# GemsLab/H2GCN

Hardware: AMD Instinct MI355X
Metric: aggregated edges/sec (1+2-hop SpMM) (higher is better)
Workload: dtype f32

## Files before the change

h2gcn_amd/csrc/spmm_kernels.hip.h:

```cpp
#pragma once

#include <hip/hip_runtime.h>
#include <stdint.h>

#include <type_traits>

#include "h2gcn_hip.h"

namespace h2gcn {

constexpr int kWave = 64;
constexpr int kWavesPerBlock = 4;
constexpr int kBlock = kWave * kWavesPerBlock;
constexpr int kNumXcd = 8;
constexpr int kMaxRowsPerWave = 7;
#ifndef H2GCN_MIN_WAVES
#define H2GCN_MIN_WAVES 6
#endif
constexpr int kMinWavesPerSimd = H2GCN_MIN_WAVES;
#ifndef H2GCN_SHORT_MIN_WAVES
#define H2GCN_SHORT_MIN_WAVES 4
#endif
#ifndef H2GCN_SHORT_FB4_MIN_WAVES
#define H2GCN_SHORT_FB4_MIN_WAVES 7
// ... 158 lines not shown
}

template <int VEC, int LPR, int NP>
__device__ __forceinline__ void fold_tree(const float (&acc)[NP][VEC], float (&tot)[VEC]) {
    constexpr int G = kWave / LPR;
    static_assert(NP == Tree<LPR>::NP, "partials per lane");
#pragma unroll
    for (int i = 0; i < VEC; ++i) {
        if constexpr (G == 1) tot[i] = (acc[0][i] + acc[1][i]) + (acc[2][i] + acc[3][i]);
        else if constexpr (G == 2) tot[i] = fold_xor32(acc[0][i]) + fold_xor32(acc[1][i]);
        else tot[i] = fold_groups<LPR>(acc[0][i]);
    }
}

template <int VEC, int NP>
__device__ __forceinline__ void zero_acc(float (&acc)[NP][VEC]) {
#pragma unroll
    for (int k = 0; k < NP; ++k)
#pragma unroll
        for (int i = 0; i < VEC; ++i) acc[k][i] = 0.f;
}

template <typename TS, int VEC>
__device__ __forceinline__ typename LoadT<TS, VEC>::type load_vec(const void* p) {
#ifdef H2GCN_NT_GATHER
    return __builtin_nontemporal_load(reinterpret_cast<const typename LoadT<TS, VEC>::type*>(p));
#else
    return *reinterpret_cast<const typename LoadT<TS, VEC>::type*>(p);
#endif
}

template <typename TS, int VEC>
__device__ __forceinline__ typename LoadT<TS, VEC>::type zero_load() {
    if constexpr (std::is_same<TS, float>::value && VEC > 1) return (typename VecT<VEC>::type)(0.f);
    else return (typename LoadT<TS, VEC>::type)0;
}

template <typename TS, int VEC>
__device__ __forceinline__ void fma_vec(float (&acc)[VEC], float w, typename LoadT<TS, VEC>::type x) {
    if constexpr (std::is_same<TS, bf16>::value) {
        if constexpr (VEC == 1) {
            acc[0] = fmaf(w, __uint_as_float((uint32_t)x << 16), acc[0]);
        } else if constexpr (VEC == 2) {
            acc[0] = fmaf(w, bf16_lo(x), acc[0]);
            acc[1] = fmaf(w, bf16_hi(x), acc[1]);
        } else {
#pragma unroll
            for (int i = 0; i < VEC / 2; ++i) {
                acc[2 * i] = fmaf(w, bf16_lo(x[i]), acc[2 * i]);
                acc[2 * i + 1] = fmaf(w, bf16_hi(x[i]), acc[2 * i + 1]);
            }
        }
    } else if constexpr (VEC == 1) {
        acc[0] = fmaf(w, x, acc[0]);
    } else {
#pragma unroll
        for (int i = 0; i < VEC; ++i) acc[i] = fmaf(w, x[i], acc[i]);
    }
}

template <bool OFF32>
struct GatherAddr {
    const char* base;
    typename std::conditional<OFF32, uint32_t, int64_t>::type lane_off;
    typename std::conditional<OFF32, uint32_t, int64_t>::type ld_bytes;
    __device__ __forceinline__ const void* row(int col) const {
        if constexpr (OFF32) {
            return base + (uint32_t)(lane_off + (uint32_t)col * ld_bytes);
        } else {
            return base + (lane_off + (int64_t)col * ld_bytes);
        }
    }
};

template <typename TS, int VEC, int LPR, int U, bool PREDICATED, bool OFF32, int PHASE = 0, int NP>
__device__ __forceinline__ void gather_batch(int c, float v, int t, int g, const GatherAddr<OFF32>& addr, bool take,
                                             float (&acc)[NP][VEC]) {
    constexpr int G = kWave / LPR;
    typename LoadT<TS, VEC>::type x[U];
    float w[U];
#pragma unroll
    for (int u = 0; u < U; ++u) {
        int cj;
        if constexpr (G == 1) {
            cj = __builtin_amdgcn_readlane(c, t + u);
            w[u] = __int_as_float(__builtin_amdgcn_readlane(__float_as_int(v), t + u));
        } else {
            const int idx = ((t + u) * G + g) & (kWave - 1);
            cj = lane_gather(c, idx);
            w[u] = lane_gather(v, idx);
        }
        const void* p = addr.row(cj);
        if constexpr (PREDICATED) {
            if (take) {
                x[u] = load_vec<TS, VEC>(p);
            } else {
                w[u] = 0.f;
                x[u] = zero_load<TS, VEC>();
            }
        } else {
            x[u] = load_vec<TS, VEC>(p);
        }
    }
#pragma unroll
    for (int u = 0; u < U; ++u) fma_vec<TS, VEC>(acc[(PHASE + u) % NP], w[u], x[u]);
}

__device__ __forceinline__ void load_chunk(const int32_t* __restrict__ colidx, const float* __restrict__ vals,
                                           int64_t base, int64_t seg_end, int lane, int& c, float& v) {
    c = 0;
    v = 0.f;
    if (base + lane < seg_end) {
        c = __builtin_nontemporal_load(colidx + base + lane);
        v = __builtin_nontemporal_load(vals + base + lane);
    }
}

template <typename TS, int VEC, int LPR, bool MASKED, bool OFF32, int MAXB = H2GCN_MAIN_MAXB, int NP>
__device__ __forceinline__ void process_chunk(int c, float v, int n, int g, const GatherAddr<OFF32>& addr,
                                              bool lane_active, float (&acc)[NP][VEC]) {
    constexpr int G = kWave / LPR;
    const int full = n / G;
    int t = 0;
    if constexpr (MAXB >= 8)
        for (; t + 8 <= full; t += 8) gather_batch<TS, VEC, LPR, 8, MASKED, OFF32>(c, v, t, g, addr, lane_active, acc);
    if constexpr (MAXB < 8)
        for (; t + 4 <= full; t += 4) gather_batch<TS, VEC, LPR, 4, MASKED, OFF32>(c, v, t, g, addr, lane_active, acc);
    if (t + 4 <= full) {
        gather_batch<TS, VEC, LPR, 4, MASKED, OFF32>(c, v, t, g, addr, lane_active, acc);
        t += 4;
    }
    const int rem = n - full * G;
    if (t + 2 <= full) {
        gather_batch<TS, VEC, LPR, 2, MASKED, OFF32>(c, v, t, g, addr, lane_active, acc);
        t += 2;
        if (t + 1 <= full) {
            gather_batch<TS, VEC, LPR, 1, MASKED, OFF32, 2 % NP>(c, v, t, g, addr, lane_active, acc);
            if constexpr (G > 1)
                if (rem > 0) gather_batch<TS, VEC, LPR, 1, true, OFF32, 3 % NP>(c, v, full, g, addr, lane_active && g < rem, acc);
        } else {
            if constexpr (G > 1)
                if (rem > 0) gather_batch<TS, VEC, LPR, 1, true, OFF32, 2 % NP>(c, v, full, g, addr, lane_active && g < rem, acc);
        }
    } else if (t + 1 <= full) {
        gather_batch<TS, VEC, LPR, 1, MASKED, OFF32>(c, v, t, g, addr, lane_active, acc);
        if constexpr (G > 1)
            if (rem > 0) gather_batch<TS, VEC, LPR, 1, true, OFF32, 1 % NP>(c, v, full, g, addr, lane_active && g < rem, acc);
    } else {
        if constexpr (G > 1)
            if (rem > 0) gather_batch<TS, VEC, LPR, 1, true, OFF32>(c, v, full, g, addr, lane_active && g < rem, acc);
    }
}

template <typename TS, int VEC, int LPR, bool MASKED, bool OFF32, int MAXB = H2GCN_MAIN_MAXB, int NP>
__device__ __forceinline__ void accumulate_segment(const int32_t* __restrict__ colidx,
                                                   const float* __restrict__ vals, int64_t seg_begin,
                                                   int64_t seg_end, int chunk0, int chunk_step,
                                                   const GatherAddr<OFF32>& addr, int lane, bool lane_active,
                                                   float (&acc)[NP][VEC]) {
    const int g = lane / LPR;
    for (int64_t base = seg_begin + (int64_t)chunk0 * kWave; base < seg_end; base += (int64_t)chunk_step * kWave) {
        const int64_t left = seg_end - base;
        const int n = left < kWave ? (int)left : kWave;
        int c;
        float v;
        load_chunk(colidx, vals, base, seg_end, lane, c, v);
        process_chunk<TS, VEC, LPR, MASKED, OFF32, MAXB>(c, v, n, g, addr, lane_active, acc);
    }
}

template <typename TS, int VEC, int LPR, bool OFF32, int MAXB = H2GCN_MAIN_MAXB, int NP>
__device__ __forceinline__ void accumulate_segment_prefetched(const int32_t* __restrict__ colidx,
                                                              const float* __restrict__ vals, int64_t seg_begin,
                                                              int64_t seg_end, int c, float v,
                                                              const GatherAddr<OFF32>& addr, int lane,
                                                              float (&acc)[NP][VEC]) {
    const int g = lane / LPR;
    for (int64_t base = seg_begin; base < seg_end; base += kWave) {
        const int64_t left = seg_end - base;
        const int n = left < kWave ? (int)left : kWave;
        int c_next = 0;
        float v_next = 0.f;
        if (left > kWave) load_chunk(colidx, vals, base + kWave, seg_end, lane, c_next, v_next);
        process_chunk<TS, VEC, LPR, false, OFF32, MAXB>(c, v, n, g, addr, true, acc);
        c = c_next;
        v = v_next;
    }
}

template <typename TS, int VEC, int LPR, bool OFF32>
__device__ __forceinline__ void accumulate_grouped(int c, float v, int n_mine, int n_max, int lane,
                                                   const GatherAddr<OFF32>& addr, float (&part)[kTreeParts][VEC]) {
    constexpr int U = kTreeParts;
    const int group_base = lane & ~(LPR - 1);
    for (int t = 0; t < n_max; t += U) {
        typename LoadT<TS, VEC>::type x[U];
        float w[U];
#pragma unroll
        for (int u = 0; u < U; ++u) {
            const int cj = lane_gather(c, group_base + t + u);
            w[u] = lane_gather(v, group_base + t + u);
            if (t + u < n_mine) {
                x[u] = load_vec<TS, VEC>(addr.row(cj));
            } else {
                w[u] = 0.f;
                x[u] = zero_load<TS, VEC>();
            }
        }
#pragma unroll
        for (int u = 0; u < U; ++u)
            if (t + u < n_mine) fma_vec<TS, VEC>(part[u], w[u], x[u]);
    }
}

template <int VEC>
__device__ __forceinline__ void combine_partials(const float (&part)[kTreeParts][VEC], float (&acc)[VEC]) {
#pragma unroll
    for (int i = 0; i < VEC; ++i) acc[i] = (part[0][i] + part[1][i]) + (part[2][i] + part[3][i]);
}

__device__ __forceinline__ float relu_keep_nan(float t) { return t < 0.f ? 0.f : t; }

template <int VEC>
__device__ __forceinline__ void epilogue(float (&acc)[VEC], const float* __restrict__ bias, int relu, int col) {
    if (bias) {
#pragma unroll
        for (int i = 0; i < VEC; ++i) acc[i] += bias[col + i];
    }
    if (relu) {
#pragma unroll
        for (int i = 0; i < VEC; ++i) acc[i] = relu_keep_nan(acc[i]);
    }
}

template <typename TD>
__device__ __forceinline__ void store_one(TD* p, float t) {
    if constexpr (std::is_same<TD, bf16>::value)
        __builtin_nontemporal_store(__builtin_bit_cast(uint16_t, (__bf16)t), reinterpret_cast<uint16_t*>(p));
    else
        __builtin_nontemporal_store(t, p);
}

template <typename TD, int VEC>
__device__ __forceinline__ void store_vec(TD* p, const float (&acc)[VEC]) {
    if constexpr (std::is_same<TD, bf16>::value) {
        if constexpr (VEC == 1) {
            store_one<TD>(p, acc[0]);
        } else if constexpr (VEC == 2) {
            __builtin_nontemporal_store(pack_bf16x2(acc[0], acc[1]), reinterpret_cast<uint32_t*>(p));
        } else {
            typename LoadT<bf16, VEC>::type o;
#pragma unroll
            for (int i = 0; i < VEC / 2; ++i) o[i] = pack_bf16x2(acc[2 * i], acc[2 * i + 1]);
            __builtin_nontemporal_store(o, reinterpret_cast<typename LoadT<bf16, VEC>::type*>(p));
        }
    } else if constexpr (VEC == 1) {
        __builtin_nontemporal_store(acc[0], p);
    } else {
        typename VecT<VEC>::type o;
#pragma unroll
        for (int i = 0; i < VEC; ++i) o[i] = acc[i];
#if defined(H2GCN_AB_NO_STORES)
        if (acc[0] == 1.2345678e30f)
            __builtin_nontemporal_store(o, reinterpret_cast<typename VecT<VEC>::type*>(p));
#elif defined(H2GCN_PLAIN_STORES)
        *reinterpret_cast<typename VecT<VEC>::type*>(p) = o;
#else
        __builtin_nontemporal_store(o, reinterpret_cast<typename VecT<VEC>::type*>(p));
#endif
    }
}

template <typename TD, int VEC, bool GEN, typename P>
__device__ __forceinline__ void store_out(const P& p, TD* row, int col0, int ecol, float (&tot)[VEC]) {
    constexpr bool kF32 = std::is_same<TD, float>::value;
    if (col0 + VEC <= p.d) {
        if constexpr (GEN) {
            if (kF32 && p.accumulate) {
                if constexpr (VEC == 1) {
                    tot[0] += reinterpret_cast<const float*>(row)[col0];
                } else {
                    const typename VecT<VEC>::type old = *reinterpret_cast<const typename VecT<VEC>::type*>(reinterpret_cast<const float*>(row) + col0);
#pragma unroll
                    for (int i = 0; i < VEC; ++i) tot[i] += old[i];
                }
            }
            epilogue<VEC>(tot, p.bias, p.relu, col0);
        }
        store_vec<TD, VEC>(row + col0, tot);
        return;
    }
    if constexpr (GEN) {
        if (col0 < p.d) {
#pragma unroll
            for (int i = 0; i < VEC; ++i) {
                const int c = ecol + i;
                if (c >= col0 && c < p.d) {
                    float t = tot[i];
                    if (kF32 && p.accumulate) t += reinterpret_cast<const float*>(row)[c];
                    if (p.bias) t += p.bias[c];
                    if (p.relu) t = relu_keep_nan(t);
                    store_one<TD>(row + c, t);
                }
            }
        }
    }
// ... 165 lines not shown
__device__ __forceinline__ void in_tile_short_rows(const LaunchParams& p, int lane, int rpw, int64_t row0, int rows_here, int rp_lo, int rp_hi,
                                                   int64_t lane_off0_, int64_t src_col_begin, int lcol, int ecol) {
    using off_t = typename std::conditional<OFF32, uint32_t, int64_t>::type;
    constexpr int NP = Tree<LPR>::NP;
    constexpr int kBias = VEC;
    const int li = lane % LPR, g = lane / LPR;
    const int n_sel = p.n_sel;
    const off_t lane_off0 = (off_t)lane_off0_;
    auto seg_bound = [&](int l) -> int64_t {
        return ((int64_t)__builtin_amdgcn_readlane(rp_hi, l) << 32) | (uint32_t)__builtin_amdgcn_readlane(rp_lo, l);
    };
    {
        constexpr int G = kWave / LPR;
        const int short_max = min(LPR, p.long_threshold - 1);
        const int n_blocks = (rows_here + G - 1) / G;
        const GatherAddr<OFF32> addr0{nullptr, lane_off0, (off_t)(p.ld_src * sizeof(TS))};
        auto row_wave_wide = [&](int r, int s_first, int s_last) {
            float acc[NP][VEC];
            zero_acc<VEC, NP>(acc);
            if constexpr (SUM) {
                for (int s = s_first; s < s_last; ++s) {
                    const int l0 = s * (rpw + 1) + r;
                    if (seg_bound(l0 + 1) - seg_bound(l0) >= p.long_threshold) return;
                }
            }
            for (int s = s_first; s < s_last; ++s) {
                const int l0 = s * (rpw + 1) + r;
                const int64_t sb = seg_bound(l0), se = seg_bound(l0 + 1);
                if (!SUM && se - sb >= p.long_threshold) continue;
                const HopCsr& h = p.hop[s];
                GatherAddr<OFF32> addr = addr0;
                addr.base = reinterpret_cast<const char*>(src_ptr<TS>(p.src) + p.src_hop_off[s] + src_col_begin - kBias);
                accumulate_segment<TS, VEC, LPR, false, OFF32, FB>(h.colidx, h.vals, sb, se, 0, 1, addr, lane, true, acc);
                if constexpr (!SUM) {
                    float tot[VEC];
                    fold_tree<VEC, LPR, NP>(acc, tot);
                    if (g == 0) store_out<TD, VEC, EPI>(p, dst_ptr<TD>(p.dst) + (row0 + r) * p.ld_dst + p.dst_hop_off[s], lcol, ecol, tot);
                    zero_acc<VEC, NP>(acc);
                }
            }
            if constexpr (SUM) {
                float tot[VEC];
                fold_tree<VEC, LPR, NP>(acc, tot);
                if (g == 0) store_out<TD, VEC, EPI>(p, dst_ptr<TD>(p.dst) + (row0 + r) * p.ld_dst, lcol, ecol, tot);
            }
        };
        auto my_segment = [&](int s, int blk, int64_t& begin, int& len) {
            const int r = blk * G + g;
            const int l0 = s * (rpw + 1) + min(r, rpw - 1);
            const int64_t sb = ((int64_t)lane_gather(rp_hi, l0) << 32) | (uint32_t)lane_gather(rp_lo, l0);
            const int64_t se = ((int64_t)lane_gather(rp_hi, l0 + 1) << 32) | (uint32_t)lane_gather(rp_lo, l0 + 1);
            begin = sb;
            const int64_t n = se - sb;
            len = r < rows_here ? (int)(n > 0x7fffffff ? 0x7fffffff : n) : -1;
        };
        if constexpr (!SUM) {
            const int n_rounds = n_sel * n_blocks;
            int64_t begin_n = 0;
            int len_n = -1, c_n = 0;
            float v_n = 0.f;
            bool short_n = false;
            auto fetch = [&](int i) {
                const int s_ = i / n_blocks, blk_ = i - s_ * n_blocks;
                my_segment(s_, blk_, begin_n, len_n);
                short_n = __builtin_amdgcn_ballot_w64(len_n > short_max) == 0;
                c_n = 0;
                v_n = 0.f;
                if (short_n && li < len_n) {
                    c_n = __builtin_nontemporal_load(p.hop[s_].colidx + begin_n + li);
                    v_n = __builtin_nontemporal_load(p.hop[s_].vals + begin_n + li);
                }
            };
            if (n_rounds > 0) fetch(0);
            for (int i = 0; i < n_rounds; ++i) {
                const int s = i / n_blocks, blk = i - s * n_blocks;
                const int len = len_n, c = c_n;
                const float v = v_n;
                const bool is_short = short_n;
                if (i + 1 < n_rounds) fetch(i + 1);
                if (is_short) {
                    int n_max = 0;
#pragma unroll
                    for (int gg = 0; gg < G; ++gg) n_max = max(n_max, __builtin_amdgcn_readlane(len, gg * LPR));
                    float part[kTreeParts][VEC];
                    zero_acc<VEC, kTreeParts>(part);
                    GatherAddr<OFF32> addr = addr0;
                    addr.base = reinterpret_cast<const char*>(src_ptr<TS>(p.src) + p.src_hop_off[s] + src_col_begin - kBias);
                    accumulate_grouped<TS, VEC, LPR, OFF32>(c, v, len, n_max, lane, addr, part);
                    float tot[VEC];
                    combine_partials<VEC>(part, tot);
                    if (len >= 0) store_out<TD, VEC, EPI>(p, dst_ptr<TD>(p.dst) + (row0 + blk * G + g) * p.ld_dst + p.dst_hop_off[s], lcol, ecol, tot);
                } else {
                    for (int gg = 0; gg < G && blk * G + gg < rows_here; ++gg) row_wave_wide(blk * G + gg, s, s + 1);
                }
            }
        } else {
            auto block_short = [&](int blk_) {
                bool ok = true;
                for (int s_ = 0; s_ < n_sel; ++s_) {
                    int64_t b_;
                    int l_;
                    my_segment(s_, blk_, b_, l_);
                    ok = ok && __builtin_amdgcn_ballot_w64(l_ > short_max) == 0;
                }
                return ok;
            };
            int64_t begin_n = 0;
            int len_n = -1, c_n = 0;
            float v_n = 0.f;
            auto fetch = [&](int blk_, int s_, bool short_blk) {
                my_segment(s_, blk_, begin_n, len_n);
                c_n = 0;
                v_n = 0.f;
                if (short_blk && li < len_n) {
                    c_n = __builtin_nontemporal_load(p.hop[s_].colidx + begin_n + li);
                    v_n = __builtin_nontemporal_load(p.hop[s_].vals + begin_n + li);
                }
            };
            bool cur_short = n_blocks > 0 && block_short(0);
            if (n_blocks > 0) fetch(0, 0, cur_short);
            for (int blk = 0; blk < n_blocks; ++blk) {
                const bool nxt_short = blk + 1 < n_blocks && block_short(blk + 1);
                if (cur_short) {
                    float part[kTreeParts][VEC];
                    zero_acc<VEC, kTreeParts>(part);
                    bool valid = false;
                    for (int s = 0; s < n_sel; ++s) {
                        const int len = len_n, c = c_n;
                        const float v = v_n;
                        valid = len >= 0;
                        if (s + 1 < n_sel) fetch(blk, s + 1, true);
                        else if (blk + 1 < n_blocks) fetch(blk + 1, 0, nxt_short);
                        int n_max = 0;
#pragma unroll
                        for (int gg = 0; gg < G; ++gg) n_max = max(n_max, __builtin_amdgcn_readlane(len, gg * LPR));
                        GatherAddr<OFF32> addr = addr0;
                        addr.base = reinterpret_cast<const char*>(src_ptr<TS>(p.src) + p.src_hop_off[s] + src_col_begin - kBias);
                        accumulate_grouped<TS, VEC, LPR, OFF32>(c, v, len, n_max, lane, addr, part);
                    }
                    float tot[VEC];
                    combine_partials<VEC>(part, tot);
                    if (valid) store_out<TD, VEC, EPI>(p, dst_ptr<TD>(p.dst) + (row0 + blk * G + g) * p.ld_dst, lcol, ecol, tot);
                } else {
                    if (blk + 1 < n_blocks) fetch(blk + 1, 0, nxt_short);
                    for (int gg = 0; gg < G && blk * G + gg < rows_here; ++gg) row_wave_wide(blk * G + gg, 0, n_sel);
                }
                cur_short = nxt_short;
            }
        }
        return;
    }
}

template <int VEC, int LPR, bool EXACT, bool SUM, bool OFF32, bool PIPE, bool SHORT, bool EPI, int FB, bool LISTS, typename TS>
constexpr int min_waves_per_simd() {
    if (!EXACT) return 2;
    if (SHORT) return FB == 4 && !SUM ? H2GCN_SHORT_FB4_MIN_WAVES : H2GCN_SHORT_MIN_WAVES;
    const bool bf16_less = std::is_same<TS, bf16>::value && VEC == 4 &&
                           (LISTS ? FB == 4 && SUM && !OFF32
                                  : (OFF32 && EPI && LPR == 32) || (SUM && OFF32 && PIPE && LPR == 16) ||
                                        (!SUM && !OFF32 && !PIPE && !EPI && LPR == 16));
    if (LISTS && FB == 4) return H2GCN_SHORT_FB4_MIN_WAVES - bf16_less;
    const bool heavy = VEC == 4 && (LISTS ? (SUM && (!OFF32 || LPR >= 32)) || (!OFF32 && LPR >= 32)
                                          : !OFF32 ? EPI || LPR >= 32 || PIPE : PIPE && LPR == 32);
    if (heavy) return H2GCN_OFF64_HEAVY_MIN_WAVES - bf16_less;
    return (LPR >= 32 ? H2GCN_WIDE_MIN_WAVES : kMinWavesPerSimd) - bf16_less;
}

template <int VEC, int LPR, bool EXACT, bool SUM, bool OFF32, bool PIPE = false, bool SHORT = false, bool EPI = false, int FB = 8, bool LISTS = false,
          typename TS = float, typename TD = float>
__global__ __launch_bounds__(kBlock, (min_waves_per_simd<VEC, LPR, EXACT, SUM, OFF32, PIPE, SHORT, EPI, FB, LISTS, TS>())) void spmm_hops_kernel(const LaunchParams p) {
    static_assert(!LISTS || (EXACT && !SHORT && !PIPE && (LPR == 16 || LPR == 32)), "list-driven launches exist for 64- and 128-column slices");
    static_assert(EXACT || LPR == kWave, "column-tiled path uses the whole wave per row");
    __shared__ float partial[kWavesPerBlock][kMaxTileCols];
    using off_t = typename std::conditional<OFF32, uint32_t, int64_t>::type;
    constexpr int NP = Tree<LPR>::NP;
    constexpr int kMainB = LISTS ? FB : (LPR >= 32 ? H2GCN_WIDE_MAXB : H2GCN_MAIN_MAXB);

    const int lane = threadIdx.x & (kWave - 1);
    const int wave = wave_uniform(threadIdx.x >> 6);
    const int li = lane % LPR;
    const int g = lane / LPR;
    const int n_sel = p.n_sel;

    const int64_t bid = blockIdx.x;
    const int slice = EXACT ? (int)(bid / p.blocks_per_slice) : 0;
    const int64_t b = EXACT ? bid - (int64_t)slice * p.blocks_per_slice : bid;
    const int col_begin = EXACT ? slice * (VEC * LPR) : 0;
    const int col_end = EXACT ? col_begin + VEC * LPR : p.d;
    const int64_t src_col_begin = EXACT ? (int64_t)slice * p.src_slice_stride : 0;
    const int lcol = col_begin + li * VEC;
    const int ecol = EXACT ? ((lcol + VEC <= p.d_src) ? lcol : p.d_src - VEC) : lcol;
    const off_t lane_off0 = (off_t)((ecol - col_begin + VEC) * (int)sizeof(TS));
    constexpr int kBias = EXACT ? VEC : 0;

    if (b < p.n_long) {
        const int64_t entry = p.long_list[b];
        const int64_t row = SUM ? entry : (entry >> 4);
        const int s_first = SUM ? 0 : (int)(entry & 15);
        const int s_last = SUM ? n_sel : s_first + 1;
        for (int col0 = col_begin; col0 < col_end; col0 += VEC * LPR) {
            const bool lane_active = EXACT || (col0 + li * VEC < p.d);
            float acc[NP][VEC];
            zero_acc<VEC, NP>(acc);
            for (int s = s_first; s < s_last; ++s) {
                const HopCsr& h = p.hop[s];
                const int64_t sb = h.rowptr[row], se = h.rowptr[row + 1];
                const GatherAddr<OFF32> addr{reinterpret_cast<const char*>(src_ptr<TS>(p.src) + p.src_hop_off[s] + src_col_begin + (col0 - col_begin) - kBias),
                                             EXACT ? lane_off0 : (off_t)(li * VEC * (int)sizeof(TS)), (off_t)(p.ld_src * sizeof(TS))};
                accumulate_segment<TS, VEC, LPR, !EXACT, OFF32, kMainB>(h.colidx, h.vals, sb, se, wave, kWavesPerBlock, addr, lane,
                                                            lane_active, acc);
            }
            float tot[VEC];
            fold_tree<VEC, LPR, NP>(acc, tot);
            if (g == 0) {
                const int rel = EXACT ? ecol - col_begin : li * VEC;
                if (!EXACT || lcol < p.d_src) {
#pragma unroll
                    for (int i = 0; i < VEC; ++i)
                        if (rel + i >= 0) partial[wave][rel + i] = tot[i];
                }
            }
            __syncthreads();
            const int c = threadIdx.x;
            if (c < VEC * LPR && col0 + c < p.d) {
                float t = partial[0][c];
#pragma unroll
                for (int w = 1; w < kWavesPerBlock; ++w) t += partial[w][c];
                const int64_t off = row * p.ld_dst + (SUM ? 0 : p.dst_hop_off[s_first]) + col0 + c;
                if constexpr (EPI) {
                    if constexpr (std::is_same<TD, float>::value)
                        if (p.accumulate) t += dst_ptr<float>(p.dst)[off];
                    if (p.bias) t += p.bias[col0 + c];
                    if (p.relu) t = relu_keep_nan(t);
                }
                store_one<TD>(dst_ptr<TD>(p.dst) + off, t);
            }
            if (!EXACT) __syncthreads();
        }
        return;
    }

    const int64_t tb = b - p.n_long;
    int64_t tile;
    if constexpr (LISTS) {
        __shared__ uint64_t s_seg[kWavesPerBlock][kShortSumHops][kWave];
        __shared__ int32_t s_row[kWavesPerBlock][kWave];
        const int64_t q = tb >> 3;
        const int i8 = (int)(tb & 7);
        const int64_t n_groups = p.short_groups + p.med_groups;
        const int64_t s_before = (q * p.short_groups) / n_groups;
        if (((q + 1) * p.short_groups) / n_groups > s_before)
            short_list_blocks<TS, TD, VEC, LPR, SUM, OFF32, EPI, H2GCN_SHORT_PREFETCH>(p, s_before * kNumXcd + i8, lane, wave, (int64_t)lane_off0,
                                                                               src_col_begin, lcol, ecol, s_seg, s_row);
        else
            medium_list_blocks<TS, TD, VEC, LPR, SUM, OFF32, EPI, FB>(p, (q - s_before) * kNumXcd + i8, lane, wave, (int64_t)lane_off0,
                                                              src_col_begin, lcol, ecol);
        return;
    } else {
        tile = (tb % kNumXcd) * p.tiles_per_xcd + tb / kNumXcd;
    }
    if (tile >= p.n_tiles) return;
    const int rpw = p.rows_per_wave;
    const int64_t row0 = (tile * kWavesPerBlock + wave) * rpw;
    if (row0 >= p.n_rows) return;
    const int64_t rows_here_l = p.n_rows - row0;
    const int rows_here = rows_here_l < rpw ? (int)rows_here_l : rpw;

    int64_t rp = 0;
    {
        const int hs = lane / (rpw + 1), r = lane % (rpw + 1);
        if (hs < n_sel && r <= rows_here) rp = p.hop[hs].rowptr[row0 + r];
    }
    const int rp_lo = (int)(rp & 0xffffffff), rp_hi = (int)(rp >> 32);
    auto seg_bound = [&](int l) -> int64_t {
        return ((int64_t)__builtin_amdgcn_readlane(rp_hi, l) << 32) | (uint32_t)__builtin_amdgcn_readlane(rp_lo, l);
    };

    if constexpr (SHORT && EXACT && (kWave / LPR == 2 || kWave / LPR == 4)) {
        in_tile_short_rows<TS, TD, VEC, LPR, SUM, OFF32, EPI, FB>(p, lane, rpw, row0, rows_here, rp_lo, rp_hi, (int64_t)lane_off0, src_col_begin, lcol, ecol);
        return;
    }
    if constexpr (PIPE && EXACT) {
        const int n_seg = rows_here * n_sel;
        uint32_t skip = 0;
        for (int q = 0; q < n_seg; ++q) {
            const int r = q / n_sel, s_ = q - r * n_sel;
            const int l0 = s_ * (rpw + 1) + r;
            if (seg_bound(l0 + 1) - seg_bound(l0) >= p.long_threshold) skip |= SUM ? (((1u << n_sel) - 1u) << (r * n_sel)) : (1u << q);
        }
        auto seg = [&](int q, int& s_, int64_t& sb, int64_t& se) {
            const int r = q / n_sel;
            s_ = q - r * n_sel;
            const int l0 = s_ * (rpw + 1) + r;
            sb = seg_bound(l0);
            se = (skip >> q) & 1u ? sb : seg_bound(l0 + 1);
        };
        int s_cur, s_nxt = 0;
        int64_t b_cur, e_cur, b_nxt = 0, e_nxt = 0;
        int c_cur, c_nxt = 0;
        float v_cur, v_nxt = 0.f;
        seg(0, s_nxt, b_nxt, e_nxt);
        load_chunk(p.hop[s_nxt].colidx, p.hop[s_nxt].vals, b_nxt, e_nxt, lane, c_nxt, v_nxt);
        float acc[NP][VEC];
        zero_acc<VEC, NP>(acc);
        for (int q = 0; q < n_seg; ++q) {
            s_cur = s_nxt; b_cur = b_nxt; e_cur = e_nxt; c_cur = c_nxt; v_cur = v_nxt;
            if (q + 1 < n_seg) {
                seg(q + 1, s_nxt, b_nxt, e_nxt);
                load_chunk(p.hop[s_nxt].colidx, p.hop[s_nxt].vals, b_nxt, e_nxt, lane, c_nxt, v_nxt);
            }
            const int r = q / n_sel;
            const int64_t row = row0 + r;
            const HopCsr& h = p.hop[s_cur];
            const GatherAddr<OFF32> addr{reinterpret_cast<const char*>(src_ptr<TS>(p.src) + p.src_hop_off[s_cur] + src_col_begin - kBias),
                                         lane_off0, (off_t)(p.ld_src * sizeof(TS))};
            accumulate_segment_prefetched<TS, VEC, LPR, OFF32>(h.colidx, h.vals, b_cur, e_cur, c_cur, v_cur, addr, lane, acc);
            const bool skipped = (skip >> q) & 1u;
            if (!SUM || s_cur == n_sel - 1) {
                if (!skipped) {
                    float tot[VEC];
                    fold_tree<VEC, LPR, NP>(acc, tot);
                    if (g == 0) store_out<TD, VEC, EPI>(p, dst_ptr<TD>(p.dst) + row * p.ld_dst + (SUM ? 0 : p.dst_hop_off[s_cur]), lcol, ecol, tot);
                }
                zero_acc<VEC, NP>(acc);
            }
        }
        return;
    }

#ifdef H2GCN_AB_STORE_BEHIND_FETCH
    if constexpr (EXACT && !SUM && !EPI) {
        float held[VEC];
        int64_t held_off = 0;
        bool held_valid = false;
        for (int r = 0; r < rows_here; ++r) {
            const int64_t row = row0 + r;
            for (int s = 0; s < n_sel; ++s) {
                const int l0 = s * (rpw + 1) + r;
                const int64_t sb = seg_bound(l0), se = seg_bound(l0 + 1);
                if (se - sb >= p.long_threshold) continue;
                const HopCsr& h = p.hop[s];
                int c;
                float v;
                load_chunk(h.colidx, h.vals, sb, se, lane, c, v);
                if (held_valid) {
                    if (g == 0) store_out<TD, VEC, EPI>(p, dst_ptr<TD>(p.dst) + held_off, lcol, ecol, held);
                    held_valid = false;
                }
                float acc[NP][VEC];
                zero_acc<VEC, NP>(acc);
                const GatherAddr<OFF32> addr{reinterpret_cast<const char*>(src_ptr<TS>(p.src) + p.src_hop_off[s] + src_col_begin - kBias), lane_off0, (off_t)(p.ld_src * sizeof(TS))};
                accumulate_segment_prefetched<TS, VEC, LPR, OFF32, kMainB>(h.colidx, h.vals, sb, se, c, v, addr, lane, acc);
                fold_tree<VEC, LPR, NP>(acc, held);
                held_off = row * p.ld_dst + p.dst_hop_off[s];
                held_valid = true;
            }
        }
        if (held_valid && g == 0) store_out<TD, VEC, EPI>(p, dst_ptr<TD>(p.dst) + held_off, lcol, ecol, held);
        return;
    }
#endif

    for (int r = 0; r < rows_here; ++r) {
        const int64_t row = row0 + r;
        if constexpr (SUM) {
            bool skip_row = false;
            for (int s = 0; s < n_sel; ++s) {
                const int l0 = s * (rpw + 1) + r;
                const int64_t len = seg_bound(l0 + 1) - seg_bound(l0);
                if (len >= p.long_threshold) skip_row = true;
            }
            if (skip_row) continue;
        }
        for (int col0 = col_begin; col0 < col_end; col0 += VEC * LPR) {
            const bool lane_active = EXACT || (col0 + li * VEC < p.d);
            float acc[NP][VEC];
            zero_acc<VEC, NP>(acc);
#ifdef H2GCN_DEFER_HOP_STORES
            float held[VEC];
            int held_s = -1;
#endif
            for (int s = 0; s < n_sel; ++s) {
                const int l0 = s * (rpw + 1) + r;
                const int64_t sb = seg_bound(l0), se = seg_bound(l0 + 1);
                if (!SUM && se - sb >= p.long_threshold) continue;
                const HopCsr& h = p.hop[s];
                const GatherAddr<OFF32> addr{reinterpret_cast<const char*>(src_ptr<TS>(p.src) + p.src_hop_off[s] + src_col_begin + (col0 - col_begin) - kBias),
                                             EXACT ? lane_off0 : (off_t)(li * VEC * (int)sizeof(TS)), (off_t)(p.ld_src * sizeof(TS))};
                accumulate_segment<TS, VEC, LPR, !EXACT, OFF32, kMainB>(h.colidx, h.vals, sb, se, 0, 1, addr, lane, lane_active, acc);
                if constexpr (!SUM) {
                    float tot[VEC];
                    fold_tree<VEC, LPR, NP>(acc, tot);
#ifdef H2GCN_DEFER_HOP_STORES
                    if (EXACT && n_sel == 2 && s == 0) {
#pragma unroll
                        for (int i = 0; i < VEC; ++i) held[i] = tot[i];
                        held_s = 0;
                    } else {
                        if (held_s >= 0 && g == 0 && lane_active)
                            store_out<TD, VEC, EPI>(p, dst_ptr<TD>(p.dst) + row * p.ld_dst + p.dst_hop_off[held_s], lcol, ecol, held);
                        held_s = -1;
                        if (g == 0 && lane_active)
                            store_out<TD, VEC, EPI>(p, dst_ptr<TD>(p.dst) + row * p.ld_dst + p.dst_hop_off[s], EXACT ? lcol : col0 + li * VEC, EXACT ? ecol : col0 + li * VEC, tot);
                    }
#else
                    if (g == 0 && lane_active)
                        store_out<TD, VEC, EPI>(p, dst_ptr<TD>(p.dst) + row * p.ld_dst + p.dst_hop_off[s], EXACT ? lcol : col0 + li * VEC, EXACT ? ecol : col0 + li * VEC, tot);
#endif
                    zero_acc<VEC, NP>(acc);
                }
            }
#ifdef H2GCN_DEFER_HOP_STORES
            if constexpr (!SUM)
                if (held_s >= 0 && g == 0 && lane_active)
                    store_out<TD, VEC, EPI>(p, dst_ptr<TD>(p.dst) + row * p.ld_dst + p.dst_hop_off[held_s], lcol, ecol, held);
#endif
            if constexpr (SUM) {
                float tot[VEC];
                fold_tree<VEC, LPR, NP>(acc, tot);
                if (g == 0 && lane_active)
                    store_out<TD, VEC, EPI>(p, dst_ptr<TD>(p.dst) + row * p.ld_dst, EXACT ? lcol : col0 + li * VEC, EXACT ? ecol : col0 + li * VEC, tot);
            }
        }
    }
}

template <bool VEC4>
__global__ void repack_slice_major_kernel(const float* __restrict__ x, int64_t ld, int64_t ld_hop, int n_hop, int64_t n_rows,
                                          int d, int n_slices, int slice_cols, float* __restrict__ w) {
    using f4 = float __attribute__((ext_vector_type(4)));
    constexpr int E = VEC4 ? 4 : 1;
    const int cu = slice_cols / E;
    const int64_t per_hop = n_rows * cu;
// ... 95 lines not shown
```

Before: 13.73 billion.

## Stage CSR column/value indices in per-wave LDS ring for 16-lane-per-row path

Adds a per-wave shared-memory ring buffer that stages interleaved (colidx, value) pairs for up to two hops. Each block of pairs is loaded with aligned 128-bit nontemporal loads and prefetched one chunk ahead of the gather loop, replacing per-chunk global loads and readlane broadcasts of neighbour indices for LPR=16 exact, non-pipelined, non-epilogue launches. It also retunes the minimum-waves-per-SIMD heuristic for the affected variants. The ring adds LDS pressure and wave barriers, and falls back to the old path when segments are too large or more than two hops are selected.

Result: faster. 13.88 billion (median of 6 runs) (+1.1%).

```diff
diff --git a/h2gcn_amd/csrc/spmm_kernels.hip.h b/h2gcn_amd/csrc/spmm_kernels.hip.h
--- a/h2gcn_amd/csrc/spmm_kernels.hip.h
+++ b/h2gcn_amd/csrc/spmm_kernels.hip.h
@@ -334,6 +334,86 @@
     }
 }
 
+constexpr int kRingHops = 2;
+constexpr int kRingCap = 256;
+constexpr int kRingBlock = 128;
+constexpr int64_t kRingMaxRange = 0x7fff0000;
+typedef uint32_t u32x2 __attribute__((ext_vector_type(2)));
+typedef uint32_t u32x4 __attribute__((ext_vector_type(4), aligned(4)));
+struct WindowChunk {
+    const uint32_t* ring;
+    uint32_t e_lane;
+    template <int G>
+    __device__ __forceinline__ void fetch(int step, int g, int& cj, float& w) const {
+        static_assert(G > 1, "the one-neighbour-per-load geometry keeps v_readlane");
+        const u32x2 pr = *reinterpret_cast<const u32x2*>(ring + 2 * ((e_lane + (uint32_t)(step * G)) & (kRingCap - 1)));
+        cj = (int)pr[0];
+        w = __uint_as_float(pr[1]);
+    }
+};
+
+template <typename TS, int VEC, int LPR, int U, bool PREDICATED, bool OFF32, int PHASE = 0, int NP>
+__device__ __forceinline__ void gather_batch_window(const WindowChunk& ch, int t, int g, const GatherAddr<OFF32>& addr, bool take,
+                                             float (&acc)[NP][VEC]) {
+    constexpr int G = kWave / LPR;
+    typename LoadT<TS, VEC>::type x[U];
+    float w[U];
+#pragma unroll
+    for (int u = 0; u < U; ++u) {
+        int cj;
+        ch.template fetch<G>(t + u, g, cj, w[u]);
+        const void* p = addr.row(cj);
+        if constexpr (PREDICATED) {
+            if (take) {
+                x[u] = load_vec<TS, VEC>(p);
+            } else {
+                w[u] = 0.f;
+                x[u] = zero_load<TS, VEC>();
+            }
+        } else {
+            x[u] = load_vec<TS, VEC>(p);
+        }
+    }
+#pragma unroll
+    for (int u = 0; u < U; ++u) fma_vec<TS, VEC>(acc[(PHASE + u) % NP], w[u], x[u]);
+}
+
+template <typename TS, int VEC, int LPR, bool MASKED, bool OFF32, int MAXB = H2GCN_MAIN_MAXB, int NP>
+__device__ __forceinline__ void process_chunk_window(const WindowChunk& ch, int n, int g, const GatherAddr<OFF32>& addr,
+                                              bool lane_active, float (&acc)[NP][VEC]) {
+    constexpr int G = kWave / LPR;
+    const int full = n / G;
+    int t = 0;
+    if constexpr (MAXB >= 8)
+        for (; t + 8 <= full; t += 8) gather_batch_window<TS, VEC, LPR, 8, MASKED, OFF32>(ch, t, g, addr, lane_active, acc);
+    if constexpr (MAXB < 8)
+        for (; t + 4 <= full; t += 4) gather_batch_window<TS, VEC, LPR, 4, MASKED, OFF32>(ch, t, g, addr, lane_active, acc);
+    if (t + 4 <= full) {
+        gather_batch_window<TS, VEC, LPR, 4, MASKED, OFF32>(ch, t, g, addr, lane_active, acc);
+        t += 4;
+    }
+    const int rem = n - full * G;
+    if (t + 2 <= full) {
+        gather_batch_window<TS, VEC, LPR, 2, MASKED, OFF32>(ch, t, g, addr, lane_active, acc);
+        t += 2;
+        if (t + 1 <= full) {
+            gather_batch_window<TS, VEC, LPR, 1, MASKED, OFF32, 2 % NP>(ch, t, g, addr, lane_active, acc);
+            if constexpr (G > 1)
+                if (rem > 0) gather_batch_window<TS, VEC, LPR, 1, true, OFF32, 3 % NP>(ch, full, g, addr, lane_active && g < rem, acc);
+        } else {
+            if constexpr (G > 1)
+                if (rem > 0) gather_batch_window<TS, VEC, LPR, 1, true, OFF32, 2 % NP>(ch, full, g, addr, lane_active && g < rem, acc);
+        }
+    } else if (t + 1 <= full) {
+        gather_batch_window<TS, VEC, LPR, 1, MASKED, OFF32>(ch, t, g, addr, lane_active, acc);
+        if constexpr (G > 1)
+            if (rem > 0) gather_batch_window<TS, VEC, LPR, 1, true, OFF32, 1 % NP>(ch, full, g, addr, lane_active && g < rem, acc);
+    } else {
+        if constexpr (G > 1)
+            if (rem > 0) gather_batch_window<TS, VEC, LPR, 1, true, OFF32>(ch, full, g, addr, lane_active && g < rem, acc);
+    }
+}
+
 template <typename TS, int VEC, int LPR, bool MASKED, bool OFF32, int MAXB = H2GCN_MAIN_MAXB, int NP>
 __device__ __forceinline__ void accumulate_segment(const int32_t* __restrict__ colidx,
                                                    const float* __restrict__ vals, int64_t seg_begin,
@@ -805,17 +885,143 @@
     }
 }
 
+template <typename T>
+__device__ __forceinline__ T pick(int s, T of_hop0, T of_hop1) { return s ? of_hop1 : of_hop0; }
+
+template <typename TS, typename TD, int VEC, int LPR, bool SUM, bool OFF32, bool EPI, int MAXB>
+__device__ __forceinline__ void window_tile_walk(const LaunchParams& p, int lane, int rpw, int64_t row0, int rows_here, int64_t rp,
+                                                 int64_t lane_off0, int64_t src_col_begin, int lcol, int ecol,
+                                                 uint32_t (&ring)[kRingHops][2 * kRingCap]) {
+    using off_t = typename std::conditional<OFF32, uint32_t, int64_t>::type;
+    constexpr int NP = Tree<LPR>::NP;
+    static_assert(kRingBlock == 4 * (kWave / 2) && kRingCap >= 2 * kRingBlock && kWave + 31 < kRingBlock, "ring safety (see above)");
+    static_assert(kRingHops == 2, "hop state is selected with pick(s, hop 0's, hop 1's)");
+    const int g = lane / LPR;
+    const int n_sel = p.n_sel;
+    const int half = lane >> 5, l4 = 4 * (lane & 31);
+    auto misalign = [](const void* a) __attribute__((always_inline)) { return (int)((reinterpret_cast<uintptr_t>(a) >> 2) & 31); };
+    const int32_t *col0 = nullptr, *col1 = nullptr;
+    const float *val0 = nullptr, *val1 = nullptr;
+    int len0 = 0, len1 = 0, mmin0 = 0, mmin1 = 0, mmax0 = 0, mmax1 = 0, blk0 = 0, blk1 = 0;
+    int rel = 0;
+    auto init_hop = [&](int s, const int32_t*& col, const float*& val, int& len, int& mmin, int& mmax) __attribute__((always_inline)) {
+        const int l0 = s * (rpw + 1);
+        const int rp_lo = (int)(rp & 0xffffffff), rp_hi = (int)(rp >> 32);
+        const int64_t org = ((int64_t)__builtin_amdgcn_readlane(rp_hi, l0) << 32) | (uint32_t)__builtin_amdgcn_readlane(rp_lo, l0);
+        if (lane >= l0) rel = (int)(rp - org);
+        len = __builtin_amdgcn_readlane(rel, l0 + rows_here);
+        col = p.hop[s].colidx + org;
+        val = p.hop[s].vals + org;
+        const int mc = misalign(col), mv = misalign(val);
+        mmin = min(mc, mv);
+        mmax = max(mc, mv);
+    };
+    init_hop(0, col0, val0, len0, mmin0, mmax0);
+    if (n_sel > 1) init_hop(1, col1, val1, len1, mmin1, mmax1);
+    auto bound = [&](int l) __attribute__((always_inline)) { return __builtin_amdgcn_readlane(rel, l); };
+    auto lane_array = [&](int s) __attribute__((always_inline)) {
+        return reinterpret_cast<const uint32_t*>(pick<const void*>(half, pick(s, col0, col1), pick(s, val0, val1)));
+    };
+    auto block_load = [&](int s, int blk) __attribute__((always_inline)) {
+        const uint32_t* a = lane_array(s);
+        const int hi = pick(s, len0, len1);
+        const int x0 = blk * kRingBlock - misalign(a) + l4;
+        u32x4 st = {0u, 0u, 0u, 0u};
+        if (x0 >= 0 && x0 + 4 <= hi) {
+            st = __builtin_nontemporal_load(reinterpret_cast<const u32x4*>(a + x0));
+        } else {
+#pragma unroll
+            for (int i = 0; i < 4; ++i)
+                if (x0 + i >= 0 && x0 + i < hi) st[i] = __builtin_nontemporal_load(a + (x0 + i));
+        }
+        return st;
+    };
+    auto block_commit = [&](int s, int blk, const u32x4& st) __attribute__((always_inline)) {
+        const int x0 = blk * kRingBlock - misalign(lane_array(s)) + l4;
+        uint32_t* slots = ring[s];
+#pragma unroll
+        for (int i = 0; i < 4; ++i) slots[2 * ((uint32_t)(x0 + i) & (kRingCap - 1)) + half] = st[i];
+        __builtin_amdgcn_fence(__ATOMIC_RELEASE, "wavefront");
+        __builtin_amdgcn_wave_barrier();
+        __builtin_amdgcn_fence(__ATOMIC_ACQUIRE, "wavefront");
+    };
+    auto blk_of = [&](int s) __attribute__((always_inline)) { return pick(s, blk0, blk1); };
+    auto set_blk = [&](int s, int b) __attribute__((always_inline)) {
+        if (s) blk1 = b;
+        else blk0 = b;
+    };
+    auto avail = [&](int s, int blk) __attribute__((always_inline)) { return blk * kRingBlock - pick(s, mmax0, mmax1); };
+
+    const int n_seg = rows_here * n_sel;
+    uint32_t skip = 0;
+    for (int q = 0; q < n_seg; ++q) {
+        const int r = q / n_sel, s_ = q - r * n_sel;
+        const int l0 = s_ * (rpw + 1) + r;
+        if (bound(l0 + 1) - bound(l0) >= p.long_threshold) skip |= SUM ? (((1u << n_sel) - 1u) << (r * n_sel)) : (1u << q);
+    }
+    float acc[NP][VEC];
+    zero_acc<VEC, NP>(acc);
+    for (int q = 0; q < n_seg; ++q) {
+        const int r = q / n_sel, s = q - r * n_sel;
+        const int l0 = s * (rpw + 1) + r;
+        const int sb = bound(l0), se = bound(l0 + 1);
+        const bool skipped = (skip >> q) & 1u;
+        if (skipped) {
+            const int b = (se + pick(s, mmin0, mmin1)) / kRingBlock;
+            if (b > blk_of(s)) set_blk(s, b);
+        } else {
+            const GatherAddr<OFF32> addr{reinterpret_cast<const char*>(src_ptr<TS>(p.src) + p.src_hop_off[s] + src_col_begin - VEC),
+                                         (off_t)lane_off0, (off_t)(p.ld_src * sizeof(TS))};
+            for (int base = sb; base < se; base += kWave) {
+                const int n = min(se - base, kWave);
+                for (int b = blk_of(s); base + n > avail(s, b); set_blk(s, ++b)) {
+                    const u32x4 st = block_load(s, b);
+                    block_commit(s, b, st);
+                }
+                int ps = s, pb = base + kWave, pe = se;
+                if (pb >= se) {
+                    pb = pe = 0;
+                    if (q + 1 < n_seg && !((skip >> (q + 1)) & 1u)) {
+                        const int r1 = (q + 1) / n_sel;
+                        ps = q + 1 - r1 * n_sel;
+                        pb = bound(ps * (rpw + 1) + r1);
+                        pe = bound(ps * (rpw + 1) + r1 + 1);
+                    }
+                }
+                const bool refill = pb < pe && min(pb + kWave, pe) > avail(ps, blk_of(ps));
+                u32x4 st = {0u, 0u, 0u, 0u};
+                if (refill) st = block_load(ps, blk_of(ps));
+                process_chunk_window<TS, VEC, LPR, false, OFF32, MAXB>(WindowChunk{ring[s], (uint32_t)(base + g)}, n, g, addr, true, acc);
+                if (refill) {
+                    block_commit(ps, blk_of(ps), st);
+                    set_blk(ps, blk_of(ps) + 1);
+                }
+            }
+        }
+        if (!SUM || s == n_sel - 1) {
+            if (!skipped) {
+                float tot[VEC];
+                fold_tree<VEC, LPR, NP>(acc, tot);
+                if (g == 0) store_out<TD, VEC, EPI>(p, dst_ptr<TD>(p.dst) + (row0 + r) * p.ld_dst + (SUM ? 0 : p.dst_hop_off[s]), lcol, ecol, tot);
+            }
+            zero_acc<VEC, NP>(acc);
+        }
+    }
+}
+
+template <int LPR, bool EXACT, bool PIPE, bool SHORT, bool EPI, bool LISTS>
+constexpr bool uses_index_window() {
+    return EXACT && !SHORT && !LISTS && !PIPE && !EPI && LPR == 16;
+}
+
 template <int VEC, int LPR, bool EXACT, bool SUM, bool OFF32, bool PIPE, bool SHORT, bool EPI, int FB, bool LISTS, typename TS>
 constexpr int min_waves_per_simd() {
     if (!EXACT) return 2;
     if (SHORT) return FB == 4 && !SUM ? H2GCN_SHORT_FB4_MIN_WAVES : H2GCN_SHORT_MIN_WAVES;
     const bool bf16_less = std::is_same<TS, bf16>::value && VEC == 4 &&
-                           (LISTS ? FB == 4 && SUM && !OFF32
-                                  : (OFF32 && EPI && LPR == 32) || (SUM && OFF32 && PIPE && LPR == 16) ||
-                                        (!SUM && !OFF32 && !PIPE && !EPI && LPR == 16));
+                           (LISTS ? FB == 4 && SUM && !OFF32 : (OFF32 && EPI && LPR == 32) || (SUM && OFF32 && PIPE && LPR == 16));
     if (LISTS && FB == 4) return H2GCN_SHORT_FB4_MIN_WAVES - bf16_less;
-    const bool heavy = VEC == 4 && (LISTS ? (SUM && (!OFF32 || LPR >= 32)) || (!OFF32 && LPR >= 32)
-                                          : !OFF32 ? EPI || LPR >= 32 || PIPE : PIPE && LPR == 32);
+    const bool heavy = VEC == 4 && (LISTS ? (SUM && (!OFF32 || LPR >= 32)) || (!OFF32 && LPR >= 32) : !OFF32 || (PIPE && LPR == 32));
     if (heavy) return H2GCN_OFF64_HEAVY_MIN_WAVES - bf16_less;
     return (LPR >= 32 ? H2GCN_WIDE_MIN_WAVES : kMinWavesPerSimd) - bf16_less;
 }
@@ -933,6 +1139,18 @@
     if constexpr (SHORT && EXACT && (kWave / LPR == 2 || kWave / LPR == 4)) {
         in_tile_short_rows<TS, TD, VEC, LPR, SUM, OFF32, EPI, FB>(p, lane, rpw, row0, rows_here, rp_lo, rp_hi, (int64_t)lane_off0, src_col_begin, lcol, ecol);
         return;
+    }
+    if constexpr (uses_index_window<LPR, EXACT, PIPE, SHORT, EPI, LISTS>()) {
+        __shared__ uint32_t ring[kWavesPerBlock][kRingHops][2 * kRingCap];
+        bool fits = n_sel <= kRingHops;
+#pragma unroll
+        for (int s = 0; s < kRingHops; ++s)
+            if (s < n_sel && seg_bound(s * (rpw + 1) + rows_here) - seg_bound(s * (rpw + 1)) > kRingMaxRange) fits = false;
+        if (fits) {
+            window_tile_walk<TS, TD, VEC, LPR, SUM, OFF32, EPI, kMainB>(p, lane, rpw, row0, rows_here, rp, (int64_t)lane_off0, src_col_begin, lcol, ecol,
+                                                                        ring[wave]);
+            return;
+        }
     }
     if constexpr (PIPE && EXACT) {
         const int n_seg = rows_here * n_sel;
```
